# Darkkey/erlamsa

Hardware: AMD Instinct MI355X
Metric: mutated_MB_per_s (higher is better)
Workload: dtype u8 (byte edits) + f64 (AS183 draws)

## Files before the change

erlamsa_amd/csrc/eh_device.h:

```cpp
#pragma once
#include <hip/hip_runtime.h>
#include <stdint.h>

#include "eh_common.h"

namespace eh {

#define EH_LANE ((int)threadIdx.x)
#define EH_DEV __device__ __forceinline__

EH_DEV uint32_t uni(uint32_t v) { return (uint32_t)__builtin_amdgcn_readfirstlane((int)v); }
EH_DEV uint64_t uni64(uint64_t v) { return ((uint64_t)uni((uint32_t)(v >> 32)) << 32) | uni((uint32_t)v); }
EH_DEV void wave_sync() { __syncthreads(); }

struct alignas(16) TabU16x65 { uint16_t v[65]; };
constexpr TabU16x65 as183_powers(uint32_t mult, uint32_t prime) {
  TabU16x65 t{};
  uint32_t a = 1;
  for (int k = 0; k <= 64; k++) { t.v[k] = (uint16_t)a; a = a * mult % prime; }
  return t;
}
__constant__ TabU16x65 c_T1 = as183_powers(171, 30269);
__constant__ TabU16x65 c_T2 = as183_powers(172, 30307);
__constant__ TabU16x65 c_T3 = as183_powers(170, 30323);
// ... 829 lines not shown
    default: return 1;
  }
}
constexpr uint32_t CODEC_WEIGHT = 64;
EH_DEV bool codec_work(Ctx& c, uint64_t bytes) {
  if (!c.work_budget) return true;
  c.work += bytes * CODEC_WEIGHT;
  if (c.work > c.work_budget) { c.status = CASE_BUDGET; return false; }
  return true;
}

EH_DEV int run_mutator_ext(Ctx& c, uint32_t fn, uint32_t mask);
EH_DEV int run_mutator(Ctx& c, uint32_t fn, uint32_t mask) {
  switch (fn) {
    case M_BD: case M_BEI: case M_BED: case M_BF: case M_BI: case M_BER: case M_BR: case M_UW: case M_UI:
      return muta_byte(c, (int)fn);
    case M_SP: case M_SR: case M_SD: case M_SNAND: case M_SRND:
      return muta_seq(c, (int)fn, (int)mask);
    case M_NIL: c.r_kind = R_SAME; return -1;
    default: return run_mutator_ext(c, fn, mask);
  }
}

EH_DEV void commit_result(Ctx& c) {
  uint32_t chunks1 = 1;
  if (c.r_flush) chunks1 = c.r_len / AVG_BLOCK_SIZE + 1;
  uint32_t chunks2 = c.r2 ? c.r2_len / AVG_BLOCK_SIZE + 1 : 0;
  uint32_t chunks = chunks1 + chunks2;
  int drop = 1 + (c.r_drop_next && c.cur + 1 < c.nb ? 1 : 0);
  int tail = c.nb - c.cur - drop;
  int newnb = c.cur + (int)chunks + tail;
  if (newnb > MAX_BLOCKS) { EH_SET_OVERFLOW(c, 104); return; }
  if (chunks != (uint32_t)drop) {
    const int l = EH_LANE;
    for (int i = l; i < tail; i += 64) c.bl2[i] = c.bl[c.cur + drop + i];
    wave_sync();
    for (int i = l; i < tail; i += 64) c.bl[c.cur + (int)chunks + i] = c.bl2[i];
  }
  for (uint32_t k = EH_LANE; k < chunks; k += 64) {
    bool second = k >= chunks1;
    uint32_t kk = second ? k - chunks1 : k, nchk = second ? chunks2 : chunks1;
    bptr base = second ? c.r2_ptr : c.r_ptr; uint32_t blen = second ? c.r2_len : c.r_len;
    bool fl = second || c.r_flush;
    uint64_t off = (uint64_t)kk * AVG_BLOCK_SIZE;
    uint32_t len = fl ? (kk + 1 < nchk ? AVG_BLOCK_SIZE : blen - (uint32_t)off) : blen;
    c.bl[c.cur + k].ptr = (uint64_t)(base + off); c.bl[c.cur + k].len = len; c.bl[c.cur + k].aux = 0;
  }
  c.nb = newnb;
  wave_sync();
}

struct alignas(16) OwnTab { uint8_t v[M_COUNT]; };
constexpr OwnTab own_atoms() {
  OwnTab t{};
  const int a[M_COUNT] = {0, 0, AT_sed_utf8_widen, AT_sed_utf8_insert, AT_ascii_bad, AT_ascii_delimeter, AT_tree_dup, AT_tree_del, AT_muta_num, AT_tree_swap_one,
                          AT_tree_stutter, AT_tree_swap_two, AT_byte_drop, AT_byte_inc, AT_byte_dec, AT_byte_flip, AT_byte_insert, AT_byte_swap_random, AT_byte_repeat,
                          AT_seq_perm, AT_seq_repeat, AT_seq_drop, AT_seq_randmask, AT_seq_randmask, AT_line_del, AT_line_del_seq, AT_line_dup, AT_line_clone,
                          AT_line_repeat, AT_line_swap, AT_line_perm, AT_list_ins, AT_list_replace, AT_fuse_this, AT_fuse_next, AT_fuse_old, AT_muta_len, 0, 0,
                          AT_muta_zippath, AT_nomutation};
  for (int i = 0; i < M_COUNT; i++) t.v[i] = (uint8_t)a[i];
  return t;
}
__constant__ OwnTab c_own_atom = own_atoms();
__device__ __noinline__ void own_meta_emit(uint32_t fn, int delta, uint32_t hlen) {
  Ctx& c = g_ctx;
  const int nm = (int)c_own_atom.v[fn];
  switch (fn) {
    case M_BD: case M_BEI: case M_BED: case M_BF: case M_BI: case M_BER: case M_BR: case M_UW: case M_UI:
    case M_FT: case M_FN: case M_FO: case M_LEN: case M_ZIP: case M_NIL:
      tr_ai(c, nm, delta); break;
    case M_SP: case M_SR: case M_SD: case M_SNAND: case M_SRND:
      tr_ai(c, nm, hlen == 0 ? -1 : (int64_t)hlen); break;
    case M_NUM: tr_ai(c, nm, c.m_aux); break;
    case M_AB: case M_AD: if (c.m_aux == 1) tr_ai(c, nm, delta); break;
    case M_LD: case M_LDS: case M_LR2: case M_LRI: case M_LR: case M_LS: case M_LP: case M_LIS: case M_LRS:
    case M_TR2: case M_TD: case M_TS1: case M_TS2: case M_TR:
      if (delta == 1) tr_ai(c, nm, 1);
      break;
    default: break;
  }
}
EH_DEV void own_meta(Ctx& c, uint32_t fn, int delta, uint32_t hlen) { if (__builtin_expect(c.trace != nullptr, 0)) own_meta_emit(fn, delta, hlen); }

constexpr uint32_t NEST_SAVE = 720;
struct MuFrame {
  uint64_t v[24];
  uint32_t pri[64], meta[64];
};
struct MxFrame {
  uint32_t e_pri[64], e_meta[64], rank[64];
  uint32_t aux_save[NEST_SAVE / 4];
  uint32_t state[64];
};

struct MxState {
  Rng rng0; uint64_t work0, mark, pt0; Blk h0;
  int32_t nfs, r, tried, j, last_tier, delta; uint32_t meta, fn, ntrace0, dropped, stateful, pad;
  uint64_t up, mu; int32_t lastm0, cur0, nb0, nfs0; uint32_t tr_base0, pad2;
};
static_assert(sizeof(MxState) % 4 == 0 && sizeof(MxState) <= 256, "MxState is copied one word per lane");
__shared__ MxState g_mx;
__device__ __noinline__ void mux_fuzzers(Ctx&, LaneTab& lt) {
  EH_CTX;
  const int l = EH_LANE;
  EH_G MxFrame* up = nullptr;
  uint32_t e_pri = lt.e_pri, e_meta = lt.e_meta, rank = 0;
  MxState& m = g_mx;
  enum { S_ENTER, S_ATTEMPT, S_RUN, S_AFTER, S_FINISH, S_LEAVE };
  int st = S_ENTER;
  for (;;) {
    if (st == S_ENTER) {
      if (c.nb - c.cur == 1 && blk_load(c.bl, c.cur).len == 0) { st = S_LEAVE; continue; }
      if (c.nb - c.cur <= 0) { c.status = CASE_CRASHED; st = S_LEAVE; continue; }
      m.nfs = c.nfs;
      uint32_t nkey = (l < m.nfs) ? em_score(e_meta) * e_pri : 0;
      unsigned long long drawing = __ballot(nkey > 0);
      uint32_t my_idx = (uint32_t)__popcll(drawing & ((1ull << l) - 1));
      uint32_t ndraw = (uint32_t)__popcll(drawing);
      uint32_t key = 0;
      if (nkey > 0) key = (uint32_t)(rng_peek(c.rng, my_idx + 1) * (double)nkey);
      rng_skip(c.rng, ndraw);
      rank = 0;
      for (int q = 0; q < m.nfs; q++) {
        uint32_t kq = (uint32_t)__builtin_amdgcn_readlane((int)key, q);
        rank += (kq > key || (kq == key && q < l)) ? 1u : 0u;
      }
#ifndef HIPEMU
      if (__builtin_readcyclecounter() - c.t_case > 20000000ull) __builtin_amdgcn_s_setprio(3);
#endif
      m.tried = 0; m.dropped = false; m.r = 0;
      m.h0 = blk_load(c.bl, c.cur);
      st = S_ATTEMPT;
    }
    if (st == S_ATTEMPT) {
      if (m.r >= m.nfs) { st = S_FINISH; continue; }
      if (m.h0.len > ABSMAX_BINARY_BLOCK) { m.dropped = true; tr_ai(c, AT_skipped_big, (int64_t)m.h0.len); st = S_FINISH; continue; }
      unsigned long long who = __ballot(l < m.nfs && rank == (uint32_t)m.r);
      m.j = (int)__builtin_ctzll(who);
      m.meta = (uint32_t)__builtin_amdgcn_readlane((int)e_meta, m.j);
      m.fn = em_fn(m.meta);
      c.r_kind = R_SAME; c.r_flush = 0; c.r_drop_next = 0; c.r_changed = 0; c.r2 = 0;
      m.mark = c.ws_used;
      if (c.work_budget) {
        c.work += (uint64_t)m.h0.len * work_weight(m.fn);
        if (c.work > c.work_budget) { c.status = CASE_BUDGET; st = S_LEAVE; continue; }
      }
#ifdef EH_PROF
      m.pt0 = __builtin_readcyclecounter();
#endif
      m.rng0 = c.rng; m.work0 = c.work; m.ntrace0 = c.ntrace;
      m.stateful = m.fn == M_LIS || m.fn == M_LRS;
      if (m.stateful) { cwptr ax = (cwptr)c.aux + (m.fn == M_LRS ? ST_STATE_WORDS : 0); for (int i = l; i < ST_STATE_WORDS; i += 64) g_st_save[i] = ax[i]; }
      m.last_tier = 0;
      c.mu_phase = 0; c.mu = nullptr;
      st = S_RUN;
    }
    if (st == S_RUN) {
      c.call_req = 0;
      m.delta = run_mutator(c, m.fn, em_mask(m.meta));
      if (c.call_req && c.status == CASE_OK) {
        EH_G MxFrame* f = nullptr;
        if (c.depth >= MAX_NEST || c.nb + 2 > MAX_BLOCKS) EH_SET_OVERFLOW(c, 301);
        else {
          f = (EH_G MxFrame*)uni64(c.mu->v[23]);
          if (!f) { f = (EH_G MxFrame*)ws_alloc(c, sizeof(MxFrame)); if (f && l == 0) c.mu->v[23] = (uint64_t)f; }
        }
        if (f) {
          EH_G uint32_t* save = f->aux_save;
          f->e_pri[l] = e_pri; f->e_meta[l] = e_meta; f->rank[l] = rank;
          EH_G uint32_t* ax = (EH_G uint32_t*)c.aux;
          for (uint32_t i = l; i < NEST_SAVE / 4; i += 64) save[i] = ax[i];
          m.up = (uint64_t)up; m.mu = (uint64_t)c.mu; m.lastm0 = c.lastm; m.tr_base0 = c.tr_base; m.cur0 = c.cur; m.nb0 = c.nb; m.nfs0 = c.nfs;
          lanes_sync();
          if ((uint32_t)l < sizeof(MxState) / 4) f->state[l] = ((const uint32_t*)&m)[l];
          wave_sync();
          if (l == 0) { ((EH_G int32_t*)c.aux)[0] = 0; ((EH_G int32_t*)(c.aux + 4 * ST_STATE_WORDS))[0] = 0; ((EH_G uint32_t*)(c.aux + 704))[3] = 0; }
          const int nb0 = c.nb;
          blk_store(c.bl, nb0, c.call_bin, c.call_len);
          e_pri = c.mu->pri[l]; e_meta = c.mu->meta[l];
          wave_sync();
          c.cur = nb0; c.nb = nb0 + 1; c.nfs = c.call_nfs; c.depth++;
          c.tr_base = c.ntrace;
          c.lex_ptr[c.depth] = 0;
          if (l == 0) lex_slot(c).n = -1;
          up = f;
          st = S_ENTER;
          continue;
        }
      }
      if (c.status == CASE_OVERFLOW && c.ovf_need != 0) {
        wave_sync();
        if (ws_regrow(c, m.mark, &m.last_tier)) {
          lex_forget_from(c, m.mark);
          c.rng = m.rng0; c.work = m.work0; c.ntrace = m.ntrace0;
          c.r_kind = R_SAME; c.r_flush = 0; c.r_drop_next = 0; c.r_changed = 0; c.r2 = 0;
          if (m.stateful) { lanes_sync(); wptr ax = (wptr)c.aux + (m.fn == M_LRS ? ST_STATE_WORDS : 0); for (int i = l; i < ST_STATE_WORDS; i += 64) ax[i] = g_st_save[i]; }
          wave_sync();
          c.mu_phase = 0; c.mu = nullptr;
          continue;
        }
      }
      st = S_AFTER;
    }
    if (st == S_AFTER) {
#ifdef EH_PROF
      if (l == 0) { atomicAdd(&c.p->prof[2 * m.fn], (unsigned long long)(__builtin_readcyclecounter() - m.pt0)); atomicAdd(&c.p->prof[2 * m.fn + 1], 1ull); }
#endif
      if (c.status != CASE_OK) { st = S_LEAVE; continue; }
      const uint32_t name = em_name(m.meta);
      uint32_t sc = em_score(m.meta);
      if (m.delta != 0) { int ns = (int)sc + m.delta; ns = ns < 2 ? 2 : (ns > 10 ? 10 : ns); sc = (uint32_t)ns; }
      uint32_t nfn = (m.fn == M_URI) ? (uint32_t)M_B64 : m.fn;
      if (l == m.j) e_meta = em_pack(sc, nfn, name, em_mask(m.meta));
      m.tried++;
      bool changed = false;
      if (c.r_kind == R_NEW) {
        wave_sync();
        uint32_t hd_len = c.r_flush && c.r_len >= AVG_BLOCK_SIZE ? AVG_BLOCK_SIZE : c.r_len;
        changed = c.r_changed || hd_len != m.h0.len || !wave_equal(c.r_ptr, (cbptr)m.h0.ptr, hd_len);
      }
#ifdef EH_PROF
    if (l == 0) {
      const unsigned long long took = c.ws_used > m.mark ? c.ws_used - m.mark : 0ull, cand = c.r_kind == R_NEW ? c.r_len : 0u;
      if (changed) { atomicAdd(&c.p->prof[2 * 57], cand); atomicAdd(&c.p->prof[2 * 57 + 1], 1ull); atomicAdd(&c.p->prof[2 * 58], took > cand ? took - cand : 0ull); atomicAdd(&c.p->prof[2 * 58 + 1], 1ull); }
      else { atomicAdd(&c.p->prof[2 * 56], took); atomicAdd(&c.p->prof[2 * 56 + 1], 1ull); }
    }
#endif
      own_meta(c, m.fn, m.delta, m.h0.len);
      tr_aa(c, changed ? AT_used : AT_failed, (int)name);
      if (changed) {
      c.lastm = (int)name;
      if (c.nchunk > 0 && m.mark <= c.ch_vstart[c.nchunk] && !c.r2) {
        int jc = c.nchunk;
        while (jc > 0 && m.mark <= c.ch_vstart[jc]) jc--;
        const uint64_t need = ((uint64_t)c.r_len + 15) & ~(uint64_t)15;
        if (m.mark + need <= c.ch_vend[jc]) {
          bptr dst = c.ch_base[jc] + m.mark;
          if (dst != c.r_ptr) {
            wave_sync();
            if (c.r_ptr > dst && c.r_ptr < dst + need) wave_move_down(dst, c.r_ptr, c.r_len); else wave_copy(dst, c.r_ptr, c.r_len);
            wave_sync();
          }
          c.r_ptr = dst;
          ws_release_to(c, m.mark);
          c.ws_used = m.mark + need;
          if (c.ws_used > c.ws_peak) c.ws_peak = c.ws_used;
        }
      }
      bptr lo = c.ws + m.mark;
      const uint64_t vs = c.ws_lo;
      if (m.mark >= vs && c.ws_used - vs > (c.ws_cap - vs) / 8 && c.r_len <= (4u << 20) && !c.r2 && c.r_ptr >= lo && c.r_ptr + c.r_len <= c.ws + c.ws_used) {
        bptr dst = lo;
        bptr hp = (bptr)m.h0.ptr;
        bool state_refs = uni(((cwptr)c.aux)[0]) != 0 || uni(((cwptr)(c.aux + 336))[0]) != 0 || uni(((cwptr)(c.aux + 704))[3]) != 0;
        if (!state_refs && hp >= c.ws + vs && hp + ((m.h0.len + 15u) & ~15u) == lo && ((uintptr_t)hp & 15) == 0) dst = hp;
        if (dst != c.r_ptr) { wave_sync(); wave_move_down(dst, c.r_ptr, c.r_len); wave_sync(); c.r_ptr = dst; }
        c.ws_used = (uint64_t)(dst - c.ws) + (((uint64_t)c.r_len + 15) & ~(uint64_t)15);
        lex_forget_from(c, (uint64_t)(dst - c.ws));
      }
        commit_result(c); st = S_FINISH; continue;
      }
      if (c.nchunk > 0) ws_release_to(c, m.mark); else c.ws_used = m.mark;
      lex_forget_from(c, m.mark);
      m.r++;
      st = S_ATTEMPT;
      continue;
    }
    if (st == S_FINISH) {
      int newpos = l;
      if (l < m.nfs) {
        int rk = (int)rank;
        if (rk < m.tried) newpos = m.tried - 1 - rk;
        else if (!m.dropped) newpos = rk;
        else newpos = rk == m.tried ? m.nfs - 1 : rk - 1;
      }
      e_meta = (uint32_t)__builtin_amdgcn_ds_permute(newpos << 2, (int)e_meta);
      e_pri = (uint32_t)__builtin_amdgcn_ds_permute(newpos << 2, (int)e_pri);
      if (m.dropped) c.nfs = m.nfs - 1;
      st = S_LEAVE;
    }
    if (!up) { lt.e_pri = e_pri; lt.e_meta = e_meta; return; }
    {
      EH_G MxFrame* f = up;
      c.depth--;
      const int nres = c.nb - c.cur;
      wave_sync();
      EH_G uint32_t* ax = (EH_G uint32_t*)c.aux; const EH_G uint32_t* save = f->aux_save;
      for (uint32_t i = l; i < NEST_SAVE / 4; i += 64) ax[i] = save[i];
      lanes_sync();
#ifdef HIPEMU
      for (uint32_t k = 0; k < sizeof(MxState) / 4; k++) ((uint32_t*)&m)[k] = f->state[k];
#else
      if ((uint32_t)l < sizeof(MxState) / 4) ((uint32_t*)&m)[l] = f->state[l];
#endif
      e_pri = f->e_pri[l]; e_meta = f->e_meta[l]; rank = f->rank[l];
      wave_sync();
      c.tr_base = m.tr_base0;
      c.cur = m.cur0; c.nb = m.nb0; c.nfs = m.nfs0; c.lastm = m.lastm0;
      c.r_kind = R_SAME; c.r_flush = 0; c.r_drop_next = 0; c.r_changed = 0; c.r2 = 0;
      c.call_nres = c.status == CASE_OK ? nres : -1;
      c.mu = (EH_G MuFrame*)m.mu; c.mu_phase = 1;
      up = (EH_G MxFrame*)m.up;
      st = S_RUN;
    }
  }
}

}
```

erlamsa_amd/csrc/eh_doc.h:

```cpp
#pragma once
#include "eh_lex.h"

namespace eh {

struct Piece { uint64_t ptr; uint32_t len; uint32_t rep; };

EH_DEV void piece_put(EH_G Piece* t, uint32_t i, const void* p, uint32_t len, uint32_t rep = 1) {
  if (EH_LANE == 0) { t[i].ptr = (uint64_t)p; t[i].len = len; t[i].rep = rep; }
}
EH_DEV uint64_t shfl64(uint64_t v, int src) { return ((uint64_t)(uint32_t)__shfl((int)(uint32_t)(v >> 32), src) << 32) | (uint32_t)__shfl((int)(uint32_t)v, src); }
EH_DEV uint32_t wave_max(uint32_t v) {
#pragma unroll
  for (int d = 32; d > 0; d >>= 1) { uint32_t t = (uint32_t)__shfl_xor((int)v, d); v = t > v ? t : v; }
  return uni(v);
}
EH_DEV uint64_t pieces_total(const EH_G Piece* t, uint32_t n) {
  uint64_t s = 0;
  for (uint32_t i = EH_LANE; i < n; i += 64) s += (uint64_t)t[i].len * t[i].rep;
  return wave_sum64(s);
}
EH_DEV uint32_t pieces_coalesce(EH_G Piece* t, uint32_t n) {
  const int l = EH_LANE;
  uint32_t nout = 0;
  uint64_t carry_end = 0; bool have_carry = false;
// ... 13 lines not shown
    bool head = valid && !cont;
    unsigned long long hm = __ballot(head);
    uint32_t hi = (uint32_t)__popcll(hm & ((2ull << l) - 1));
    uint32_t len = valid ? p.len : 0u;
    uint32_t inc = wave_incl_scan(len);
    unsigned long long after = hm & ~((2ull << l) - 1);
    int endl = after ? (int)__builtin_ctzll(after) - 1 : 63;
    uint32_t run_total = (uint32_t)__shfl((int)inc, endl) - (inc - len);
    wave_sync();
    if (head) { Piece q; q.ptr = p.ptr; q.len = run_total; q.rep = p.rep; t[nout + hi - 1] = q; }
    uint32_t first_head = hm ? (uint32_t)__builtin_ctzll(hm) : 64u;
    uint32_t carry_add = first_head > 0 ? (uint32_t)__builtin_amdgcn_readlane((int)inc, (int)(first_head - 1)) : 0u;
    if (carry_add > 0 && l == 0 && nout > 0) t[nout - 1].len += carry_add;
    nout += (uint32_t)__popcll(hm);
    if (vm) {
      int last = 63 - (int)__builtin_clzll(vm);
      carry_end = readlane64(p.ptr + p.len, (uint32_t)last);
      have_carry = __shfl((int)(plain ? 1 : 0), last) != 0;
    }
    wave_sync();
  }
  return nout;
}
EH_DEV void wave_gather(bptr dst, const EH_G Piece* t, uint32_t n) {
  const int l = EH_LANE;
  uint64_t pos = 0;
  for (uint32_t base = 0; base < n; base += 64) {
    uint32_t idx = base + (uint32_t)l;
    uint64_t ptr = 0; uint32_t len = 0, rep = 1;
    if (idx < n) { Piece p = t[idx]; ptr = p.ptr; len = p.len; rep = p.rep; }
    uint64_t tl = (uint64_t)len * rep;
    uint64_t inc = tl;
#pragma unroll
    for (int d = 1; d < 64; d <<= 1) {
      uint64_t up = ((uint64_t)(uint32_t)__shfl_up((int)(uint32_t)(inc >> 32), d) << 32) | (uint32_t)__shfl_up((int)(uint32_t)inc, d);
      if (l >= d) inc += up;
    }
    uint64_t off = pos + inc - tl;
    bool big = len > 48 || rep > 1;
    uint32_t maxs = wave_max(big ? 0u : len);
    cbptr sp = (cbptr)ptr;
    bptr dp = dst + off;
    for (uint32_t i0 = 0; i0 < maxs; i0 += 8) {
      uint8_t b[8];
#pragma unroll
      for (uint32_t k = 0; k < 8; k++) if (!big && i0 + k < len) b[k] = sp[i0 + k];
#pragma unroll
      for (uint32_t k = 0; k < 8; k++) if (!big && i0 + k < len) dp[i0 + k] = b[k];
    }
    unsigned long long bm = __ballot(big && tl > 0);
    while (bm) {
      int j = (int)__builtin_ctzll(bm); bm &= bm - 1;
      uint64_t pj = readlane64(ptr, (uint32_t)j), oj = readlane64(off, (uint32_t)j);
      uint32_t lj = (uint32_t)__builtin_amdgcn_readlane((int)len, j), rj = (uint32_t)__builtin_amdgcn_readlane((int)rep, j);
      if (rj == 1) wave_copy(dst + oj, (cbptr)pj, lj);
      else wave_fill_periodic(dst + oj, (cbptr)pj, lj, (uint64_t)lj * rj);
    }
    pos += readlane64(inc, 63);
  }
}
EH_DEV void pieces_append(EH_G Piece* dst, uint32_t* n, const EH_G Piece* src, uint32_t a, uint32_t b) {
  if (b <= a) return;
  uint32_t cnt = b - a, at = *n;
  for (uint32_t i = EH_LANE; i < cnt; i += 64) dst[at + i] = src[a + i];
  *n = at + cnt;
}
EH_DEV bool pieces_materialize(Ctx& c, const EH_G Piece* t, uint32_t a, uint32_t b, bptr* out, uint32_t* outlen) {
  wave_sync();
  uint64_t tot = pieces_total(t + a, b - a);
  if (tot > 0xFFFFFFF0ull) { EH_SET_OVERFLOW(c, 201); return false; }
  bptr d = ws_alloc(c, tot ? tot : 16);
  if (!d) return false;
  wave_gather(d, t + a, b - a);
  wave_sync();
  *out = d; *outlen = (uint32_t)tot;
  return true;
}
struct IsInk { EH_DEV bool operator()(uint32_t b, uint32_t) const { return b != 0 && b != 10 && b != 13 && b != 32; } };

EH_DEV EH_G MuFrame* mu_frame(Ctx& c) {
  if (c.mu) return c.mu;
  EH_G MuFrame* m = (EH_G MuFrame*)ws_alloc(c, sizeof(MuFrame));
  if (m && EH_LANE == 0) m->v[23] = 0;
  c.mu = m;
  return m;
}

__constant__ uint8_t c_def_pri[M_COUNT] = {10, 3, 1, 2, 1, 1, 1, 1, 3, 2, 2, 2, 1, 1, 1, 1, 1, 1, 1, 1, 1, 1, 1, 1, 1, 1, 1, 1, 1, 1, 1, 1, 1, 2, 1, 2, 2, 7, 1, 1, 0};

EH_DEV void inner_table(Ctx& c, bool json, EH_G MuFrame* mu, int* nfs) {
  const int l = EH_LANE;
  (void)rng_rand(c.rng, 3); (void)rng_rand(c.rng, 1);
  const uint8_t sg[11] = {M_AB, M_AD, M_NUM, M_BD, M_SD, M_LD, M_LRI, M_LR, M_LP, M_B64, M_URI};
  const uint8_t js[9] = {M_SGM, M_AB, M_AD, M_NUM, M_SP, M_SR, M_SD, M_B64, M_URI};
  int n = json ? 9 : 11;
  uint32_t name = 0;
#pragma unroll
  for (int k = 0; k < 11; k++) if (k == l) name = json ? (k < 9 ? js[k] : 0) : sg[k];
  uint32_t score = 0;
  if (l < n) { uint32_t v = (uint32_t)(rng_peek(c.rng, (uint32_t)(n - 1 - l) + 1) * 10.0); score = v < 2 ? 2 : v; }
  rng_skip(c.rng, (uint64_t)n);
  mu->pri[l] = l < n ? (uint32_t)c_def_pri[name] : 0;
  mu->meta[l] = em_pack(score, name, name, 3u);
  *nfs = n;
}

__device__ __noinline__ int muta_b64(Ctx&, EH_G LexCache& lc) {
  EH_CTX;
  const int l = EH_LANE;
  Blk hb = blk_load(c.bl, c.cur);
  cbptr H = (cbptr)hb.ptr; uint32_t L = hb.len;
  c.r_kind = R_SAME;
  EH_G LexChunk* tab = nullptr;
  int n = 0, base = 0, dacc = -1, d = 0;
  uint32_t snand_mask = 0, nout = 0, cap = 0, done_to = 0, a = 0, b = 0;
  unsigned long long cand = 0;
  EH_G Piece* out = nullptr;
  bool resume = c.mu_phase == 1;
  EH_G MuFrame* mu = c.mu;
  EH_PT0;
  if (!resume) {
    n = lex_cached(c, lc, H, L, &tab);
    if (n < 0) return 0;
    EH_PT(c, 48);
    snand_mask = rng_rand(c.rng, 3); (void)rng_rand(c.rng, 1);
  } else {
    tab = (EH_G LexChunk*)uni64(mu->v[0]); n = (int)uni((uint32_t)mu->v[1]); base = (int)uni((uint32_t)mu->v[2]); cand = uni64(mu->v[3]);
    snand_mask = uni((uint32_t)mu->v[4]); nout = uni((uint32_t)mu->v[5]); cap = uni((uint32_t)mu->v[6]); done_to = uni((uint32_t)mu->v[7]);
    a = uni((uint32_t)mu->v[8]); b = uni((uint32_t)mu->v[9]); dacc = (int)uni((uint32_t)mu->v[10]); d = (int)uni((uint32_t)mu->v[11]);
    out = (EH_G Piece*)uni64(mu->v[12]);
  }
  for (; base < n; base += 64) {
   int ti = base + l;
   uint32_t cty = 1, ca = 0, cb = 0;
   if (ti < n) { LexChunk e = tab[ti]; cty = e.type; ca = e.a; cb = e.b; }
   if (!resume) cand = __ballot(cty == 0 && cb - ca > 6);
   while (cand || resume) {
    if (!resume) {
      int cj = (int)__builtin_ctzll(cand); cand &= cand - 1;
      a = (uint32_t)__builtin_amdgcn_readlane((int)ca, cj); b = (uint32_t)__builtin_amdgcn_readlane((int)cb, cj);
      uint32_t nalpha, span;
      if (!b64_accepts(H + a, b - a, &nalpha, &span)) continue;
      uint32_t dl = b64_decoded_len(nalpha);
      if (!out) {
        cap = 2 * (uint32_t)(n - (base + cj)) + 4;
        out = (EH_G Piece*)ws_alloc(c, (uint64_t)cap * sizeof(Piece));
        if (!out) return 0;
      }
      if (!mu) { mu = mu_frame(c); if (!mu) return 0; }
      bptr dec = ws_alloc(c, (uint64_t)dl + 16);
      bptr pack = nalpha != span ? ws_alloc(c, (uint64_t)nalpha + 16) : nullptr;
      if (!dec || (nalpha != span && !pack)) return 0;
      EH_PT(c, 49);
      b64_decode_wave(H + a, span, nalpha, dec, pack);
      wave_sync();
      EH_PT(c, 50);
      d = rng_delta(c.rng);
      tr_ai(c, AT_base64_mutator, d);
      uint32_t name = l < (int)M_COUNT ? (uint32_t)((int)M_COUNT - 1 - l) : 0;
      uint32_t score = 0;
      if (l < (int)M_COUNT) { uint32_t v = (uint32_t)(rng_peek(c.rng, name + 1) * 10.0); score = v < 2 ? 2 : v; }
      rng_skip(c.rng, (uint64_t)M_COUNT);
      mu->pri[l] = l < (int)M_COUNT ? (uint32_t)c_def_pri[name] : 0;
      mu->meta[l] = em_pack(score, name, name, name == M_SNAND ? snand_mask : 3u);
      if (l == 0) {
        mu->v[0] = (uint64_t)tab; mu->v[1] = (uint32_t)n; mu->v[2] = (uint32_t)base; mu->v[3] = cand; mu->v[4] = snand_mask; mu->v[5] = nout; mu->v[6] = cap;
        mu->v[7] = done_to; mu->v[8] = a; mu->v[9] = b; mu->v[10] = (uint32_t)dacc; mu->v[11] = (uint32_t)d; mu->v[12] = (uint64_t)out;
      }
      wave_sync();
      c.call_req = 1; c.call_bin = (uint64_t)dec; c.call_len = dl; c.call_nfs = (int)M_COUNT;
      return 0;
    }
    resume = false;
    const int nres = c.call_nres;
    if (nres < 0) return 0;
    EH_PT(c, 51);
    uint64_t tot = 0;
    for (int k = 0; k < nres; k++) tot += blk_load(c.bl, c.nb + k).len;
    if (tot > 0xBFFFFFF0ull) { EH_SET_OVERFLOW(c, 202); return 0; }
    bptr nb = ws_alloc(c, tot + 16);
    bptr enc = ws_alloc(c, (tot + 2) / 3 * 4 + 16);
    if (!nb || !enc) return 0;
    uint64_t o = 0;
    for (int k = 0; k < nres; k++) { Blk x = blk_load(c.bl, c.nb + k); wave_copy(nb + o, (cbptr)x.ptr, x.len); o += x.len; }
    wave_sync();
    b64_encode(nb, (uint32_t)tot, enc);
    wave_sync();
    piece_put(out, nout, H + done_to, a - done_to); nout++;
    piece_put(out, nout, enc, (uint32_t)((tot + 2) / 3 * 4)); nout++;
    done_to = b;
    dacc += d;
    EH_PT(c, 52);
   }
  }
  EH_PT(c, 49);
  if (!out) return -1;
  piece_put(out, nout, H + done_to, L - done_to); nout++;
  wave_sync();
  uint64_t total = pieces_total(out, nout);
  if (total > 0xFFFFFFF0ull) { EH_SET_OVERFLOW(c, 203); return 0; }
  bptr dst = ws_alloc(c, total ? total : 16);
  if (!dst) return 0;
  wave_gather(dst, out, nout);
  wave_sync();
  EH_PT(c, 53);
  c.r_kind = R_NEW; c.r_ptr = dst; c.r_len = (uint32_t)total;
  return dacc;
}

}
```

erlamsa_amd/csrc/eh_lex.h:

```cpp
#pragma once
#include "eh_text.h"
#include "eh_mask.h"

namespace eh {

struct ByteReader {
  cbptr p; uint32_t n; uint32_t wbase; uint32_t w; bool valid;
};
EH_DEV void br_init(ByteReader& r, cbptr p, uint32_t n) { r.p = p; r.n = n; r.wbase = 0; r.w = 0; r.valid = false; }
EH_DEV void br_fill(ByteReader& r, uint32_t from) {
  r.wbase = from;
  uint32_t off = from + 4u * (uint32_t)EH_LANE;
  uint32_t v = 0;
  if (off + 4 <= r.n) v = ldg4(r.p + off);
  else { for (uint32_t k = 0; k < 4; k++) if (off + k < r.n) v |= (uint32_t)r.p[off + k] << (8 * k); }
  r.w = v; r.valid = true;
}
EH_DEV uint32_t br_get(ByteReader& r, uint32_t i, uint32_t hint) {
  if (!r.valid || i < r.wbase || i >= r.wbase + 256) br_fill(r, hint);
  uint32_t d = i - r.wbase;
  uint32_t word = (uint32_t)__builtin_amdgcn_readlane((int)r.w, (int)uni(d >> 2));
  return (word >> (8 * (d & 3))) & 255u;
}

// ... 273 lines not shown
    uint32_t b = p[i0 + k];
    if (pred(b, hist & 0xFFFFFFu)) m |= 1u << k;
    hist = (hist << 8) | b;
  }
  return m;
}
struct IsUriSep { EH_DEV bool operator()(uint32_t b, uint32_t h) const { return b == '/' && (h & 0xFFFF) == ((uint32_t)':' << 8 | '/'); } };
struct IsEocd { EH_DEV bool operator()(uint32_t b, uint32_t h) const { return b == 0x06 && h == (0x50u << 16 | 0x4Bu << 8 | 0x05u); } };

EH_DEV bool has_zip_eocd(cbptr H, uint32_t L) {
  if (L < 22) return false;
  uint32_t lo = L > 22 + 65535 ? L - 22 - 65535 : 0;
  uint32_t found = 0;
  for (uint32_t tb = lo & ~1023u; tb < L; tb += 1024) {
    uint32_t m = tile_mask_h(H, L, tb, IsEocd());
    uint32_t mm = m;
    while (mm) { uint32_t bit = (uint32_t)__builtin_ctz(mm); mm &= mm - 1; uint32_t e = tb + 16u * (uint32_t)EH_LANE + bit; if (e >= 3 && e - 3 >= lo && e - 3 + 22 <= L) found = 1; }
  }
  return __ballot(found != 0) != 0;
}
EH_DEV bool b64_accepts(cbptr t, uint32_t n, uint32_t* nalpha_out, uint32_t* span_out) {
  const int l = EH_LANE;
  uint32_t nalpha = 0, eqpos = 0xFFFFFFFFu;
  for (uint32_t base = 0; base < n && eqpos == 0xFFFFFFFFu; base += 64) {
    uint32_t i = base + (uint32_t)l; bool in = i < n;
    uint32_t ch = in ? t[i] : 32u;
    bool ws = ch == 9 || ch == 10 || ch == 13 || ch == 32;
    bool al = (ch >= 'A' && ch <= 'Z') || (ch >= 'a' && ch <= 'z') || (ch >= '0' && ch <= '9') || ch == '+' || ch == '/';
    unsigned long long em = __ballot(in && ch == '='), om = __ballot(in && !ws && !al && ch != '='), am = __ballot(in && al);
    unsigned long long upto = em ? ((1ull << __builtin_ctzll(em)) - 1) : ~0ull;
    if (om & upto) return false;
    nalpha += (uint32_t)__popcll(am & upto);
    if (em) eqpos = base + (uint32_t)__builtin_ctzll(em);
  }
  uint32_t q = nalpha & 3u;
  *nalpha_out = nalpha; *span_out = eqpos == 0xFFFFFFFFu ? n : eqpos;
  if (eqpos == 0xFFFFFFFFu) return q == 0;
  if (q != 2 && q != 3) return false;
  uint32_t need = q == 2 ? 1u : 0u; bool ok = true;
  for (uint32_t base = eqpos + 1; base < n && ok; base += 64) {
    uint32_t i = base + (uint32_t)l; bool in = i < n;
    uint32_t ch = in ? t[i] : 32u;
    bool ws = ch == 9 || ch == 10 || ch == 13 || ch == 32;
    unsigned long long nm = __ballot(in && !ws);
    while (nm && ok) {
      int j = (int)__builtin_ctzll(nm); nm &= nm - 1;
      uint32_t cj = (uint32_t)__builtin_amdgcn_readlane((int)ch, j);
      if (need && cj == '=') need = 0; else ok = false;
    }
  }
  return ok && need == 0;
}
EH_DEV uint32_t b64_decoded_len(uint32_t nalpha) { uint32_t q = nalpha & 3u; return nalpha / 4 * 3 + (q == 2 ? 1u : (q == 3 ? 2u : 0u)); }
EH_DEV uint32_t b64_sextet(uint32_t ch) {
  return ch >= 'a' ? ch - 'a' + 26 : (ch >= 'A' ? ch - 'A' : (ch >= '0' ? ch - '0' + 52 : (ch == '+' ? 62u : 63u)));
}
EH_DEV void b64_decode_wave(cbptr t, uint32_t span, uint32_t nalpha, bptr dst, bptr pack) {
  const int l = EH_LANE;
  cbptr src = t;
  if (nalpha != span) {
    uint32_t cnt = 0;
    for (uint32_t base = 0; base < span; base += 64) {
      uint32_t i = base + (uint32_t)l; bool in = i < span;
      uint32_t ch = in ? t[i] : 32u;
      bool al = in && !(ch == 9 || ch == 10 || ch == 13 || ch == 32);
      unsigned long long am = __ballot(al);
      if (al) pack[cnt + (uint32_t)__popcll(am & ((1ull << l) - 1))] = (uint8_t)ch;
      cnt += (uint32_t)__popcll(am);
    }
    wave_sync();
    src = pack;
  }
  uint32_t ng = nalpha / 4, q = nalpha & 3u;
  for (uint32_t g = (uint32_t)l; g < ng; g += 64) {
    uint32_t v = (b64_sextet(src[4 * g]) << 18) | (b64_sextet(src[4 * g + 1]) << 12) | (b64_sextet(src[4 * g + 2]) << 6) | b64_sextet(src[4 * g + 3]);
    dst[3 * g] = (uint8_t)(v >> 16); dst[3 * g + 1] = (uint8_t)(v >> 8); dst[3 * g + 2] = (uint8_t)v;
  }
  if (l == 63 && q >= 2) {
    uint32_t v = (b64_sextet(src[4 * ng]) << 6) | b64_sextet(src[4 * ng + 1]);
    if (q == 2) dst[3 * ng] = (uint8_t)(v >> 4);
    else { v = (v << 6) | b64_sextet(src[4 * ng + 2]); dst[3 * ng] = (uint8_t)(v >> 10); dst[3 * ng + 1] = (uint8_t)(v >> 2); }
  }
}
EH_DEV void b64_encode(cbptr src, uint32_t n, bptr dst) {
  uint32_t ng = (n + 2) / 3;
  for (uint32_t g = EH_LANE; g < ng; g += 64) {
    uint32_t i = 3 * g, rem = n - i;
    uint32_t b0 = src[i], b1 = rem > 1 ? src[i + 1] : 0, b2 = rem > 2 ? src[i + 2] : 0;
    uint32_t v = (b0 << 16) | (b1 << 8) | b2;
    auto ch = [](uint32_t x) -> uint8_t { return (uint8_t)(x < 26 ? 'A' + x : (x < 52 ? 'a' + (x - 26) : (x < 62 ? '0' + (x - 52) : (x == 62 ? '+' : '/')))); };
    dst[4 * g] = ch((v >> 18) & 63); dst[4 * g + 1] = ch((v >> 12) & 63);
    dst[4 * g + 2] = rem > 1 ? ch((v >> 6) & 63) : (uint8_t)'=';
    dst[4 * g + 3] = rem > 2 ? ch(v & 63) : (uint8_t)'=';
  }
}
__device__ __noinline__ int muta_uri(Ctx&, EH_G LexCache& lc) {
  EH_CTX;
  Blk hb = blk_load(c.bl, c.cur);
  cbptr H = (cbptr)hb.ptr; uint32_t L = hb.len;
  c.r_kind = R_SAME;
  EH_G LexChunk* tab;
  int n = lex_cached(c, lc, H, L, &tab);
  if (n < 0) return 0;
  uint32_t nsep = 0;
  for (uint32_t tb = 0; tb < L; tb += 1024) nsep += __popc(tile_mask_h(H, L, tb, IsUriSep()));
  nsep = wave_sum(nsep);
  if (nsep == 0) return -1;
  const DevConfig& cfg = c.p->cfg;
  uint32_t hostlen = 0; while (cfg.ssrf_host[hostlen]) hostlen++;
  uint64_t bound = (uint64_t)L + (uint64_t)nsep * (hostlen + 96) + 64;
  bptr dst = ws_alloc(c, bound);
  if (!dst) return 0;
  uint32_t out = 0; int dacc = -1; bool crashed = false;
  auto copy_range = [&](uint32_t a, uint32_t b) { wave_copy(dst + out, H + a, b - a); out += b - a; };
  for (int i = 0; i < n && !crashed; i++) {
    LexChunk e = tab[i];
    uint32_t ty = uni(e.type), a = uni(e.a), b = uni(e.b);
    if (ty != 0 || b - a <= 5) { copy_range(a, b); continue; }
    uint32_t sp = 0xFFFFFFFFu;
    if (EH_LANE == 0) { for (uint32_t k = a; k + 2 < b; k++) if (H[k] == ':' && H[k + 1] == '/' && H[k + 2] == '/') { sp = k; break; } }
    sp = uni((uint32_t)__shfl((int)sp, 0));
    if (sp == 0xFFFFFFFFu) { copy_range(a, b); continue; }
    uint32_t tstart = sp + 3;
    uint32_t mode = rng_erand(c.rng, 3);
    bool file_scheme = sp - a >= 4 && uni(H[sp - 4]) == 'f' && uni(H[sp - 3]) == 'i' && uni(H[sp - 2]) == 'l' && uni(H[sp - 1]) == 'e';
    uint32_t dom_a = 0, dom_b = 0; bool have_dom = false;
    if (mode != 1) {
      uint32_t da = 0, db = 0, hv = 0;
      if (EH_LANE == 0) { uint32_t k = tstart; while (k < b && H[k] == '/') k++; if (k < b) { hv = 1; da = k; while (k < b && H[k] != '/') k++; db = k; } }
      dom_a = uni((uint32_t)__shfl((int)da, 0)); dom_b = uni((uint32_t)__shfl((int)db, 0)); have_dom = uni((uint32_t)__shfl((int)hv, 0)) != 0;
    }
    uint32_t at_sp = 0, ntrav = 0, which = 0;
    if (mode == 2) at_sp = rng_rand(c.rng, 2);
    if (mode != 1 && !have_dom) { crashed = true; break; }
    if (mode == 3) { ntrav = rng_erand(c.rng, 10); which = rng_erand(c.rng, 4); }
    wave_sync();
    uint32_t newout = out;
    if (EH_LANE == 0) {
      uint32_t o = out;
      auto putb = [&](uint8_t v) { dst[o++] = v; };
      auto puts = [&](const char* s) { while (*s) dst[o++] = (uint8_t)*s++; };
      auto putr = [&](uint32_t x, uint32_t y) { for (uint32_t k = x; k < y; k++) dst[o++] = H[k]; };
      auto put_query_joined = [&]() {
        uint32_t k = dom_b; bool first = true;
        while (k < b) { while (k < b && H[k] == '/') k++; if (k >= b) break; if (!first) putb('/'); first = false; while (k < b && H[k] != '/') putb(H[k++]); }
      };
      if (mode == 1) {
        if (file_scheme) { putr(a, sp - 4); puts("http"); } else putr(a, sp);
        puts("://"); puts(cfg.ssrf_host); putb(':'); puts(cfg.ssrf_port); putb('/');
        putr(tstart, b);
      } else if (mode == 2) {
        if (file_scheme) { putr(a, sp - 4); puts("http"); } else putr(a, sp);
        puts("://"); putr(dom_a, dom_b);
        if (at_sp == 0) putb(' ');
        putb('@'); puts(cfg.ssrf_host); putb(':'); puts(cfg.ssrf_port);
        putb('/'); put_query_joined();
      } else {
        putr(a, sp); puts("://"); putr(dom_a, dom_b);
        putb('/'); for (uint32_t k = 0; k < ntrav; k++) puts("../");
        if (which == 1) put_query_joined(); else if (which == 2) puts("Windows/win.ini"); else if (which == 3) puts("etc/shadow"); else puts("etc/passwd");
      }
      newout = o;
    }
    out = uni((uint32_t)__shfl((int)newout, 0));
    dacc += 1;
    tr_aa(c, AT_uri, AT_success);
    wave_sync();
  }
  if (crashed) { c.status = CASE_CRASHED; return 0; }
  wave_sync();
  c.r_kind = R_NEW; c.r_ptr = dst; c.r_len = out;
  return dacc;
}

}
```

include/erlamsa_hip.h:

```cpp
#ifndef ERLAMSA_HIP_H
#define ERLAMSA_HIP_H
#include <stdint.h>
#ifdef __cplusplus
extern "C" {
#endif

#define EH_ABI_VERSION 8

typedef struct eh_ctx eh_ctx;

enum eh_error {
  EH_OK = 0,
  EH_E_INVALID = -1,
  EH_E_NODEVICE = -2,
  EH_E_HIP = -3,
  EH_E_NOMEM = -4,
  EH_E_STATE = -5,
  EH_E_UNSUPPORTED = -6,
  EH_E_AGAIN = -7
};

enum eh_case_status {
  EH_CASE_OK = 0,
  EH_CASE_CRASHED = 1,
  EH_CASE_OVERFLOW = 2,
  EH_CASE_UNSUPPORTED = 3,
  EH_CASE_ARENA_FULL = 4,
  EH_CASE_BUDGET = 5
};

typedef struct eh_options {
  uint32_t abi_version;
  const char* mutations;
  const char* patterns;
  const char* generators;
  double blockscale;
  const char* ssrf_host;
  int32_t ssrf_port;
  uint64_t max_case_bytes;
  uint64_t out_capacity;
  uint64_t max_case_work;
  uint32_t max_slots;
  uint32_t flags;
  uint64_t big_case_bytes;
  uint64_t pool_bytes;
  uint64_t download_chunk_bytes;
  uint64_t fuse_stream_min;
  uint32_t sequence_muta;
  uint32_t reserved0;
} eh_options;

#define EH_FLAG_NO_COOP 64u
#define EH_FLAG_TREE_NO_LANES 128u
#define EH_FLAG_ORDERED_OUTPUT 1u
#define EH_FLAG_META_TRACE 2u
#define EH_FLAG_SGML_NO_LANES 32u
#define EH_FLAG_SGML_NO_REPLAY 16u
#define EH_FLAG_FUSE_NO_REDUCE 8u
#define EH_FLAG_FUSE_NO_LDS 4u

int eh_create(int device, eh_ctx** out);
void eh_destroy(eh_ctx* ctx);
int eh_configure(eh_ctx* ctx, const eh_options* opts);

int eh_corpus_upload(eh_ctx* ctx, const uint8_t* data, const uint64_t* off, uint64_t n);
int eh_corpus_attach(eh_ctx* ctx, const void* d_data, const void* d_off, uint64_t n, uint64_t nbytes);

int eh_device_count(void);
int eh_comm_unique_id(uint8_t id[128]);
int eh_comm_init(eh_ctx* ctx, const uint8_t id[128], int rank, int nranks);
int eh_comm_init_local(eh_ctx** ctxs, int nctx);
int eh_comm_destroy(eh_ctx* ctx);
int eh_corpus_broadcast(eh_ctx* ctx, int root, const uint8_t* data, const uint64_t* off, uint64_t n);
int eh_corpus_allgather(eh_ctx* ctx, const uint8_t* data, const uint64_t* off, uint64_t n_local);
int eh_corpus_broadcast_local(eh_ctx** ctxs, int nctx, int root);

int eh_corpus_device(eh_ctx* ctx, const void** d_data, const void** d_off, uint64_t* n, uint64_t* nbytes);

int eh_stream(eh_ctx* ctx, void** stream);

int eh_host_alloc(void** p, uint64_t bytes);
void eh_host_free(void* p);

int eh_reserve(eh_ctx* ctx, uint64_t max_cases);

int eh_fuzz_batch(eh_ctx* ctx, const int64_t seed[3], uint64_t first_case, uint64_t corpus_first, uint64_t n,
                  void* stream);
int eh_fuzz_calls(eh_ctx* ctx, const int64_t* seeds, uint64_t corpus_first, uint64_t n, void* stream);
int eh_sync(eh_ctx* ctx);
int eh_batch_done(eh_ctx* ctx, int* done);

int eh_coalesce_limits(eh_ctx* ctx, uint64_t flush_cases, uint64_t flush_bytes);
int eh_submit(eh_ctx* ctx, const uint8_t* data, uint64_t len, const int64_t seed[3], uint64_t* ticket);
int eh_flush(eh_ctx* ctx);
int eh_poll(eh_ctx* ctx, uint64_t ticket, uint8_t* out, uint64_t cap, uint64_t* out_len, int32_t* status);
int eh_cancel(eh_ctx* ctx, uint64_t ticket);

#define EH_MAX_PROFILES 1024
int eh_profile_add(eh_ctx* ctx, const char* mutations, const char* patterns, double blockscale, uint32_t* id);
int eh_profile_count(eh_ctx* ctx, uint32_t* n);
int eh_fuzz_calls_profiled(eh_ctx* ctx, const int64_t* seeds, const uint32_t* profile, uint64_t corpus_first, uint64_t n, void* stream);
int eh_submit_profiled(eh_ctx* ctx, const uint8_t* data, uint64_t len, const int64_t seed[3], uint32_t profile, uint64_t* ticket);

int eh_result_device(eh_ctx* ctx, const uint8_t** d_data, const uint64_t** d_off, const uint64_t** d_len,
                     const int32_t** d_status, uint64_t* total_bytes);
int eh_result_download(eh_ctx* ctx, uint8_t* data, uint64_t cap, uint64_t* off, int32_t* status);
int eh_result_fetch(eh_ctx* ctx, uint64_t i, uint8_t* buf, uint64_t cap, uint64_t* out_len);
int eh_result_totals(eh_ctx* ctx, uint64_t* in_bytes, uint64_t* out_bytes, uint64_t* n_cases);
int eh_result_summary(eh_ctx* ctx, uint64_t* out);
int eh_result_occupancy(eh_ctx* ctx, uint64_t* out);
int eh_result_diag(eh_ctx* ctx, uint64_t* draws, int32_t* last_mutator);

int eh_result_cycles(eh_ctx* ctx, uint64_t* cycles);

int eh_result_write_files(eh_ctx* ctx, const char* name_template, uint64_t first_number, uint32_t threads,
                          uint64_t* files_written, uint64_t* bytes_written, uint64_t* not_written);

int eh_meta_atom_count(void);
const char* eh_meta_atom_name(int id);
int eh_result_meta(eh_ctx* ctx, uint64_t i, uint8_t* buf, uint64_t cap, uint64_t* n_events);

#define EH_UNIQUE_PIECE_BYTES 65536
int eh_result_digests(eh_ctx* ctx, uint64_t* digest);
int eh_result_unique(eh_ctx* ctx, uint64_t* first_of, uint64_t* n_unique, uint64_t* unique_bytes);
int eh_result_download_select(eh_ctx* ctx, const uint64_t* idx, uint64_t m, uint8_t* data, uint64_t cap, uint64_t* off);
int eh_selftest_unique(eh_ctx* ctx, const uint8_t* data, const uint64_t* off, const int32_t* status, uint64_t n,
                       uint64_t* digest, uint64_t* first_of);

int eh_result_peak(eh_ctx* ctx, uint64_t* peak);

int eh_result_prof(eh_ctx* ctx, uint64_t* prof);

int eh_selftest_movers(eh_ctx* ctx, uint8_t* buf, uint64_t buf_len, const uint32_t* jobs, uint32_t njobs, uint32_t* eq_out);
int eh_selftest_zlib(eh_ctx* ctx, int op, const uint8_t* in, uint64_t n, uint8_t* out, uint64_t cap, uint64_t* out_len, int32_t* ok);

int eh_selftest_sort_by_priority(const uint32_t* pri, uint32_t n, uint32_t* perm);
// ... 25 lines not shown
```

Baseline: 79610.

## Skip redundant nest frame saves, encode base64 in place with SWAR bulk path

```diff
diff --git a/erlamsa_amd/csrc/eh_device.h b/erlamsa_amd/csrc/eh_device.h
--- a/erlamsa_amd/csrc/eh_device.h
+++ b/erlamsa_amd/csrc/eh_device.h
@@ -935,6 +935,12 @@
 }
 EH_DEV void own_meta(Ctx& c, uint32_t fn, int delta, uint32_t hlen) { if (__builtin_expect(c.trace != nullptr, 0)) own_meta_emit(fn, delta, hlen); }
 
+#ifdef HIPEMU
+extern "C" { inline unsigned long long eh_emu_nested[6] = {0, 0, 0, 0, 0, 0}; }
+#define NEST_COUNT(i, v) do { if (EH_LANE == 0) eh_emu_nested[i] += (v); } while (0)
+#else
+#define NEST_COUNT(i, v) do { } while (0)
+#endif
 constexpr uint32_t NEST_SAVE = 720;
 struct MuFrame {
   uint64_t v[24];
@@ -944,6 +950,9 @@
   uint32_t e_pri[64], e_meta[64], rank[64];
   uint32_t aux_save[NEST_SAVE / 4];
   uint32_t state[64];
+#ifdef EH_PROF
+  uint64_t t_enter;
+#endif
 };
 
 struct MxState {
@@ -1012,21 +1021,41 @@
       c.call_req = 0;
       m.delta = run_mutator(c, m.fn, em_mask(m.meta));
       if (c.call_req && c.status == CASE_OK) {
+        EH_PT0;
         EH_G MxFrame* f = nullptr;
+        bool fresh = false;
         if (c.depth >= MAX_NEST || c.nb + 2 > MAX_BLOCKS) EH_SET_OVERFLOW(c, 301);
         else {
           f = (EH_G MxFrame*)uni64(c.mu->v[23]);
-          if (!f) { f = (EH_G MxFrame*)ws_alloc(c, sizeof(MxFrame)); if (f && l == 0) c.mu->v[23] = (uint64_t)f; }
+          if (!f) { fresh = true; f = (EH_G MxFrame*)ws_alloc(c, sizeof(MxFrame)); if (f && l == 0) c.mu->v[23] = (uint64_t)f; }
         }
         if (f) {
           EH_G uint32_t* save = f->aux_save;
-          f->e_pri[l] = e_pri; f->e_meta[l] = e_meta; f->rank[l] = rank;
           EH_G uint32_t* ax = (EH_G uint32_t*)c.aux;
-          for (uint32_t i = l; i < NEST_SAVE / 4; i += 64) save[i] = ax[i];
-          m.up = (uint64_t)up; m.mu = (uint64_t)c.mu; m.lastm0 = c.lastm; m.tr_base0 = c.tr_base; m.cur0 = c.cur; m.nb0 = c.nb; m.nfs0 = c.nfs;
-          lanes_sync();
-          if ((uint32_t)l < sizeof(MxState) / 4) f->state[l] = ((const uint32_t*)&m)[l];
-          wave_sync();
+          NEST_COUNT(4, 1);
+#ifdef HIPEMU
+          if (l == 0 && (unsigned long long)(c.depth + 1) > eh_emu_nested[3]) eh_emu_nested[3] = (unsigned long long)(c.depth + 1);
+#endif
+          if (fresh || (c.p->flags & EH_FLAG_NEST_PLAIN)) {
+            NEST_COUNT(0, 1);
+            f->e_pri[l] = e_pri; f->e_meta[l] = e_meta; f->rank[l] = rank;
+            for (uint32_t i = l; i < NEST_SAVE / 4; i += 64) save[i] = ax[i];
+            m.up = (uint64_t)up; m.mu = (uint64_t)c.mu; m.lastm0 = c.lastm; m.tr_base0 = c.tr_base; m.cur0 = c.cur; m.nb0 = c.nb; m.nfs0 = c.nfs;
+            lanes_sync();
+            if ((uint32_t)l < sizeof(MxState) / 4) f->state[l] = ((const uint32_t*)&m)[l];
+            wave_sync();
+          } else {
+            NEST_COUNT(1, 1);
+#ifdef HIPEMU
+            unsigned long long bad = (f->e_pri[l] != e_pri) + (f->e_meta[l] != e_meta) + (f->rank[l] != rank);
+            for (uint32_t i = l; i < NEST_SAVE / 4; i += 64) bad += save[i] != ax[i];
+            MxState t = m;
+            t.up = (uint64_t)up; t.mu = (uint64_t)c.mu; t.lastm0 = c.lastm; t.tr_base0 = c.tr_base; t.cur0 = c.cur; t.nb0 = c.nb; t.nfs0 = c.nfs;
+            if ((uint32_t)l < sizeof(MxState) / 4 && (uint32_t)l != offsetof(MxState, delta) / 4) bad += f->state[l] != ((const uint32_t*)&t)[l];
+            eh_emu_nested[2] += bad;
+            wave_sync();
+#endif
+          }
           if (l == 0) { ((EH_G int32_t*)c.aux)[0] = 0; ((EH_G int32_t*)(c.aux + 4 * ST_STATE_WORDS))[0] = 0; ((EH_G uint32_t*)(c.aux + 704))[3] = 0; }
           const int nb0 = c.nb;
           blk_store(c.bl, nb0, c.call_bin, c.call_len);
@@ -1038,6 +1067,10 @@
           if (l == 0) lex_slot(c).n = -1;
           up = f;
           st = S_ENTER;
+          EH_PT(c, 44);
+#ifdef EH_PROF
+          if (l == 0) f->t_enter = pt_;
+#endif
           continue;
         }
       }
@@ -1135,6 +1168,7 @@
     if (!up) { lt.e_pri = e_pri; lt.e_meta = e_meta; return; }
     {
       EH_G MxFrame* f = up;
+      EH_PT0;
       c.depth--;
       const int nres = c.nb - c.cur;
       wave_sync();
@@ -1155,8 +1189,11 @@
       c.mu = (EH_G MuFrame*)m.mu; c.mu_phase = 1;
       up = (EH_G MxFrame*)m.up;
       st = S_RUN;
-    }
-  }
-}
-
-}
+#ifdef EH_PROF
+      { const uint64_t t0_ = pt_, te_ = uni64(f->t_enter); EH_PT(c, 45); if (l == 0) { atomicAdd(&c.p->prof[2 * 46], (unsigned long long)(t0_ - te_)); atomicAdd(&c.p->prof[2 * 46 + 1], 1ull); } }
+#endif
+    }
+  }
+}
+
+}
diff --git a/erlamsa_amd/csrc/eh_doc.h b/erlamsa_amd/csrc/eh_doc.h
--- a/erlamsa_amd/csrc/eh_doc.h
+++ b/erlamsa_amd/csrc/eh_doc.h
@@ -119,6 +119,7 @@
   if (c.mu) return c.mu;
   EH_G MuFrame* m = (EH_G MuFrame*)ws_alloc(c, sizeof(MuFrame));
   if (m && EH_LANE == 0) m->v[23] = 0;
+  if (m) NEST_COUNT(5, 1);
   c.mu = m;
   return m;
 }
@@ -206,23 +207,43 @@
       }
       wave_sync();
       c.call_req = 1; c.call_bin = (uint64_t)dec; c.call_len = dl; c.call_nfs = (int)M_COUNT;
+      EH_PT(c, 47);
       return 0;
     }
     resume = false;
     const int nres = c.call_nres;
     if (nres < 0) return 0;
     EH_PT(c, 51);
-    uint64_t tot = 0;
-    for (int k = 0; k < nres; k++) tot += blk_load(c.bl, c.nb + k).len;
+    uint64_t tot = 0, first = 0; bool gaps = false;
+    for (int k0 = 0; k0 < nres; k0 += 64) {
+      const int k = k0 + l;
+      uint64_t p = 0, pn = 0; uint32_t ln = 0;
+      if (k < nres) { p = c.bl[c.nb + k].ptr; ln = c.bl[c.nb + k].len; }
+      if (k + 1 < nres) pn = c.bl[c.nb + k + 1].ptr;
+      tot += ln;
+      gaps |= k + 1 < nres && p + ln != pn;
+      if (k0 == 0) first = readlane64(p, 0);
+    }
+    tot = wave_sum64(tot);
+    const bool in_place = !__ballot(gaps) && !(c.p->flags & EH_FLAG_NEST_PLAIN);
+    EH_PT(c, 41);
     if (tot > 0xBFFFFFF0ull) { EH_SET_OVERFLOW(c, 202); return 0; }
-    bptr nb = ws_alloc(c, tot + 16);
+    cbptr src = (cbptr)first;
+    if (!in_place) {
+      bptr nb = ws_alloc(c, tot + 16);
+      if (!nb) return 0;
+      uint64_t o = 0;
+      for (int k = 0; k < nres; k++) { Blk x = blk_load(c.bl, c.nb + k); wave_copy(nb + o, (cbptr)x.ptr, x.len); o += x.len; }
+      wave_sync();
+      src = nb;
+      EH_PT(c, 42);
+    }
     bptr enc = ws_alloc(c, (tot + 2) / 3 * 4 + 16);
-    if (!nb || !enc) return 0;
-    uint64_t o = 0;
-    for (int k = 0; k < nres; k++) { Blk x = blk_load(c.bl, c.nb + k); wave_copy(nb + o, (cbptr)x.ptr, x.len); o += x.len; }
-    wave_sync();
-    b64_encode(nb, (uint32_t)tot, enc);
-    wave_sync();
+    if (!enc) return 0;
+    const bool plain = (c.p->flags & EH_FLAG_NEST_PLAIN) != 0;
+    b64_encode(src, (uint32_t)tot, enc, !plain);
+    if (plain) wave_sync();
+    EH_PT(c, 43);
     piece_put(out, nout, H + done_to, a - done_to); nout++;
     piece_put(out, nout, enc, (uint32_t)((tot + 2) / 3 * 4)); nout++;
     done_to = b;
diff --git a/erlamsa_amd/csrc/eh_lex.h b/erlamsa_amd/csrc/eh_lex.h
--- a/erlamsa_amd/csrc/eh_lex.h
+++ b/erlamsa_amd/csrc/eh_lex.h
@@ -379,16 +379,43 @@
     else { v = (v << 6) | b64_sextet(src[4 * ng + 2]); dst[3 * ng] = (uint8_t)(v >> 10); dst[3 * ng + 1] = (uint8_t)(v >> 2); }
   }
 }
-EH_DEV void b64_encode(cbptr src, uint32_t n, bptr dst) {
+EH_DEV uint32_t b64_chars(uint32_t v) {
+  const uint32_t x = ((v >> 18) & 63u) | (((v >> 12) & 63u) << 8) | (((v >> 6) & 63u) << 16) | ((v & 63u) << 24);
+  auto ge = [&](uint32_t t) -> uint32_t { return ((x + (128u - t) * 0x01010101u) >> 7) & 0x01010101u; };
+  return x + 65u * 0x01010101u + 6u * ge(26) - 75u * ge(52) - 15u * ge(62) + 3u * ge(63);
+}
+EH_DEV void b64_encode(cbptr src, uint32_t n, bptr dst, bool bulk = true) {
+  uint32_t g0 = 0;
+  if (bulk && ((uintptr_t)dst & 15) == 0) {
+    const uint32_t nu = n / 12;
+    for (uint32_t u0 = 0; u0 < nu; u0 += 256) {
+      uint32_t w[4][3] = {};
+#pragma unroll
+      for (int j = 0; j < 4; j++) {
+        const uint32_t u = u0 + 64u * (uint32_t)j + (uint32_t)EH_LANE;
+        if (u < nu) { cbptr s = src + 12ull * u; w[j][0] = ldg4(s); w[j][1] = ldg4(s + 4); w[j][2] = ldg4(s + 8); }
+      }
+#pragma unroll
+      for (int j = 0; j < 4; j++) {
+        const uint32_t u = u0 + 64u * (uint32_t)j + (uint32_t)EH_LANE;
+        if (u >= nu) continue;
+        const uint32_t a = __builtin_bswap32(w[j][0]), b = __builtin_bswap32(w[j][1]), d = __builtin_bswap32(w[j][2]);
+        uint4 o;
+        o.x = b64_chars(a >> 8); o.y = b64_chars(((a & 0xFFu) << 16) | (b >> 16)); o.z = b64_chars(((b & 0xFFFFu) << 8) | (d >> 24)); o.w = b64_chars(d & 0xFFFFFFu);
+        stg16a(dst + 16ull * u, o);
+      }
+    }
+    g0 = 4 * nu;
+  }
   uint32_t ng = (n + 2) / 3;
-  for (uint32_t g = EH_LANE; g < ng; g += 64) {
+  for (uint32_t g = g0 + EH_LANE; g < ng; g += 64) {
     uint32_t i = 3 * g, rem = n - i;
     uint32_t b0 = src[i], b1 = rem > 1 ? src[i + 1] : 0, b2 = rem > 2 ? src[i + 2] : 0;
     uint32_t v = (b0 << 16) | (b1 << 8) | b2;
-    auto ch = [](uint32_t x) -> uint8_t { return (uint8_t)(x < 26 ? 'A' + x : (x < 52 ? 'a' + (x - 26) : (x < 62 ? '0' + (x - 52) : (x == 62 ? '+' : '/')))); };
-    dst[4 * g] = ch((v >> 18) & 63); dst[4 * g + 1] = ch((v >> 12) & 63);
-    dst[4 * g + 2] = rem > 1 ? ch((v >> 6) & 63) : (uint8_t)'=';
-    dst[4 * g + 3] = rem > 2 ? ch(v & 63) : (uint8_t)'=';
+    uint32_t q = b64_chars(v);
+    dst[4 * g] = (uint8_t)q; dst[4 * g + 1] = (uint8_t)(q >> 8);
+    dst[4 * g + 2] = rem > 1 ? (uint8_t)(q >> 16) : (uint8_t)'=';
+    dst[4 * g + 3] = rem > 2 ? (uint8_t)(q >> 24) : (uint8_t)'=';
   }
 }
 __device__ __noinline__ int muta_uri(Ctx&, EH_G LexCache& lc) {
diff --git a/include/erlamsa_hip.h b/include/erlamsa_hip.h
--- a/include/erlamsa_hip.h
+++ b/include/erlamsa_hip.h
@@ -52,6 +52,7 @@
 
 #define EH_FLAG_NO_COOP 64u
 #define EH_FLAG_TREE_NO_LANES 128u
+#define EH_FLAG_NEST_PLAIN 256u
 #define EH_FLAG_ORDERED_OUTPUT 1u
 #define EH_FLAG_META_TRACE 2u
 #define EH_FLAG_SGML_NO_LANES 32u
```

Result: no change. 80710, median of 3 (+1.4%).
